# fallenshock/SinDDM

Hardware: AMD Instinct MI355X
Metric: diffusion steps/sec (finest scale) + imgs/sec full multi-scale sample, 1/2/4/8 GPU (higher is better)
Workload: dtype f32 (3x3 convs: binary16 hi/lo split products -- Winograd-domain GEMMs with all 4 MFMA terms, fp32 accumulate; fp32-equivalent, error vs float64 = the fp32 oracle's: tests/test_gpu_h2.py; everything else fp32); 1 GPU; C3: 6-scale pyramid, T=1000, finest scale 411x512, batch 64 per GPU, dim=160; batch_per_gpu=64, global_batch=64, scale=5, parallelism=independent chains over 1 GPU(s), one all-gather of the images

## Files before the change

include/sinddm_hip_debug.h:

```cpp
#ifndef SINDDM_HIP_DEBUG_H
#define SINDDM_HIP_DEBUG_H

#include <stddef.h>
#include <stdint.h>

#ifdef __cplusplus
extern "C" {
#endif

int sinddm_prof_begin(void);
int sinddm_prof_end(double* conv_ms_total, int64_t* conv_launches, double* conv_flops_total);
int sinddm_prof_end2(double* conv_ms_total, int64_t* conv_launches, double* conv_flops_total,
                     double* conv_exec_flops_total);
int sinddm_prof_end3(int kind, double* ms_total, int64_t* launches, double* flops_total,
                     double* exec_flops_total, int reset);

int sinddm_debug_routes(int dim_arg, int train, int B, int H, int W, int out[16]);

#define SINDDM_FWD_PLAN_BLOCK0 24
#define SINDDM_FWD_PLAN_BLOCK_INTS 14
#define SINDDM_FWD_PLAN_INTS (SINDDM_FWD_PLAN_BLOCK0 + 4 * SINDDM_FWD_PLAN_BLOCK_INTS)
#define SINDDM_FWD_PLAN_INTS_EXT (SINDDM_FWD_PLAN_INTS + 4)
int sinddm_debug_forward_plan(int dim_arg, int train, int B, int H, int W, int ncu, int64_t* out, int cap);

int sinddm_debug_first_conv(int variant, int ncu, int B, int H, int W, int Wt, int Cout, const float* in, const float* weights,
                            const float* bias, float* out, float* amax_out, void* stream);

int sinddm_debug_conv_path(int dim, int B, int H, int W);

int sinddm_debug_infer_path(int dim, int B, int H, int W);

int sinddm_debug_head_path(int dim, int B, int H, int W);
int sinddm_debug_head_offsets(int dim, int64_t out[3]);
int sinddm_debug_head(const float* packed, const float* g, const float* x_in, float* eps_out, int dim, int B, int H, int W,
                      int Wp, void* stream);

int sinddm_debug_train_path(int dim, int B, int H, int W);

int sinddm_debug_conv_wh(int variant, int ncu, int B, int H, int W, int Wt, int Cin, int Cout, int act, const float* in,
                         const float* weights, const float* bias, const float* resid, const float* aux, float* out,
                         float* out_pre, float* amax_out, void* scratch, size_t scratch_bytes, void* stream);
size_t sinddm_debug_conv_wh_scratch_bytes(int Cin, int Cout, int B);

int sinddm_debug_block_train(const float* params, const float* packed, const float* packed_bwd, int dim, int l,
                             const float* x, const float* cond_bias, const float* grad_y, float* y, float* grad_x,
                             float* grad_params, float* dcond, int B, int H, int W, void* ws, size_t ws_bytes,
                             void* stream);

int sinddm_debug_wgrad_map(int Cin, int Cout, int64_t ntiles, int ncu, uint32_t* wg_out, int wg_cap, int32_t* splits_out,
                           int splits_cap);

#define SINDDM_DWGRAD_TILES 6
#define SINDDM_DWGRAD_ROWS 7
int sinddm_debug_wgrad_plan(int taps, int Cin, int Cout, int B, int H, int W, int have_scr, int have_amax, int ncu, int out[4]);
int sinddm_debug_wgrad(int taps, int Cin, int Cout, int B, int H, int W, int ncu, int have_scr, int use_amax, const float* dout,
                       const float* in, float* gw, float* gb, void* scratch, size_t scratch_bytes, int plan_out[4], void* stream);
size_t sinddm_debug_wgrad_scratch_bytes(int taps, int Cin, int Cout, int B);
int sinddm_debug_wgrad_routes(int dim_arg, int B, int H, int W, int ncu, int* out, int cap);

// ... 5 lines not shown
```

sinddm_amd/_lib.py:

```python
from __future__ import annotations

import ctypes as C
import os
from typing import Optional

import torch

_HERE = os.path.dirname(os.path.abspath(__file__))
LIB_PATH = os.path.join(_HERE, "libsinddm_hip.so")

ABI_SYMBOLS = (
    "sinddm_abi_version", "sinddm_param_count", "sinddm_param_tensors", "sinddm_param_offset",
    "sinddm_packed_count", "sinddm_workspace_bytes", "sinddm_pack_weights", "sinddm_net_forward",
    "sinddm_q_sample", "sinddm_reverse_step", "sinddm_reverse_step_edit", "sinddm_upsample_bilinear", "sinddm_prof_begin", "sinddm_prof_end", "sinddm_prof_end2", "sinddm_prof_end3", "sinddm_debug_wgrad_map", "sinddm_debug_conv_path",
    "sinddm_debug_block_train", "sinddm_debug_infer_path", "sinddm_debug_train_path",
    "sinddm_train_workspace_bytes", "sinddm_packed_bwd_count", "sinddm_pack_weights_bwd",
    "sinddm_net_forward_train", "sinddm_net_backward", "sinddm_l1_loss_fwd_bwd", "sinddm_adam_ema_step",
    "sinddm_cond_embed", "sinddm_cond_stride", "sinddm_sample_chain", "sinddm_sample_chain2", "sinddm_sample_chain_ex",
    "sinddm_normal_fill", "sinddm_wrap_halo", "sinddm_upsample_bilinear_wrap", "sinddm_sample_chain_tile",
    "sinddm_sample_chain_keep", "sinddm_reverse_step_keep", "sinddm_normal_fill_samples", "sinddm_sample_chain_seeds",
    "sinddm_debug_head_path", "sinddm_debug_head_offsets", "sinddm_debug_head", "sinddm_debug_routes",
    "sinddm_debug_forward_plan",
    "sinddm_debug_wgrad_routes", "sinddm_debug_wgrad_plan", "sinddm_debug_wgrad", "sinddm_debug_wgrad_scratch_bytes",
    "sinddm_sample_chain_resample", "sinddm_reverse_step_jump",
    "sinddm_sample_chain_layout", "sinddm_layout_delta", "sinddm_reverse_step_layout",
    "sinddm_sample_chain_batch",
    "sinddm_sample_chain_solver", "sinddm_reverse_step_ms",
    "sinddm_q_sample_wrap", "sinddm_l1_loss_crop_fwd_bwd",
    "sinddm_sample_chain_mix", "sinddm_normal_fill_mix",
    "sinddm_l1_loss_weighted_fwd_bwd",
    "sinddm_debug_conv_wh", "sinddm_debug_conv_wh_scratch_bytes",
    "sinddm_debug_first_conv",
    "sinddm_patch_nnf_workspace_bytes", "sinddm_patch_nnf",
    "sinddm_q_sample_crop", "sinddm_l1_loss_rect_fwd_bwd",
    "sinddm_sample_chain_gate", "sinddm_reverse_step_keep_gate",
    "sinddm_patch_nnf_scaled_workspace_bytes", "sinddm_patch_nnf_scaled", "sinddm_patch_vote",
    "sinddm_score_workspace_bytes", "sinddm_score_chain",
    "sinddm_normal_fill_window",
)


ABI_VERSION = 3
DIM_FP32_CONVS = 0x10000
JUMP_STREAM = 1 << 31
MIX_MAX = 4
SCORE_MAX_EVALS = 1024
TILE_HALO = 16


class StepCoefs(C.Structure):
    _fields_ = [("mode", C.c_int), ("clip", C.c_int),
                ("sqrt_recip_ac_t", C.c_float), ("sqrt_recipm1_ac_t", C.c_float),
                ("coef1_t", C.c_float), ("coef2_t", C.c_float),
                ("gamma_t", C.c_float), ("gamma_tm1", C.c_float),
                ("sqrt_ac_tm1", C.c_float), ("sqrt_ac_t", C.c_float), ("sqrt_1m_ac_t", C.c_float),
                ("sqrt_1m_ac_tm1_mvar", C.c_float), ("sigma", C.c_float)]


class ChainOpts(C.Structure):
    _fields_ = [("edit_w", C.c_void_p), ("edit_c", C.c_void_p), ("noise", C.c_void_p)]


class KeepOpts(C.Structure):
    _fields_ = [("mask", C.c_void_p), ("x0", C.c_void_p), ("ab", C.POINTER(C.c_float))]

# ... 95 lines not shown
        "sinddm_normal_fill_window": (i, [p, i, p, i, i, i, p, i, i, p, p, i, p]),
        "sinddm_reverse_step_ms": (i, [p, p, p, p, p, C.POINTER(StepCoefs), f, p, p, p, p, p, f, f, i, i, i, p]),
        "sinddm_layout_delta": (i, [p, p, p, p, p, C.POINTER(StepCoefs), p, p, i, i, i, i, i, i, p]),
        "sinddm_reverse_step_layout": (i, [p, p, p, p, p, C.POINTER(StepCoefs), p, f, i, p, p, p, p, f, f, i, i, i, i, i, i, i,
                                           p]),
        "sinddm_reverse_step_jump": (i, [p, p, p, p, p, p, C.POINTER(StepCoefs), C.POINTER(JumpCoefs), p, p, p, p, f, f, i, i, i,
                                         p]),
        "sinddm_normal_fill_samples": (i, [p, i, i64, p, C.c_uint64, p]),
        "sinddm_reverse_step_keep": (i, [p, p, p, p, p, C.POINTER(StepCoefs), p, p, p, p, f, f, i, i, i, p]),
        "sinddm_reverse_step_keep_gate": (i, [p, p, p, p, p, C.POINTER(StepCoefs), p, p, p, p, f, f, i, i, i, p, f]),
        "sinddm_wrap_halo": (i, [p, p, i, i, i, i, i, p]),
        "sinddm_upsample_bilinear_wrap": (i, [p, p, i, i, i, i, i, i, i, p]),
        "sinddm_normal_fill": (i, [p, i64, C.c_uint64, C.c_uint64, p]),
        "sinddm_upsample_bilinear": (i, [p, p, i, i, i, i, i, p]),
        "sinddm_prof_begin": (i, []),
        "sinddm_prof_end": (i, [C.POINTER(C.c_double), C.POINTER(C.c_int64), C.POINTER(C.c_double)]),
        "sinddm_prof_end2": (i, [C.POINTER(C.c_double), C.POINTER(C.c_int64), C.POINTER(C.c_double),
                                 C.POINTER(C.c_double)]),
        "sinddm_prof_end3": (i, [i, C.POINTER(C.c_double), C.POINTER(C.c_int64), C.POINTER(C.c_double),
                                 C.POINTER(C.c_double), i]),
        "sinddm_debug_wgrad_map": (i, [i, i, i64, i, C.POINTER(C.c_uint32), i, C.POINTER(C.c_int32), i]),
        "sinddm_debug_conv_path": (i, [i, i, i, i]),
        "sinddm_debug_infer_path": (i, [i, i, i, i]),
        "sinddm_debug_train_path": (i, [i, i, i, i]),
        "sinddm_debug_head_path": (i, [i, i, i, i]),
        "sinddm_debug_routes": (i, [i, i, i, i, i, C.POINTER(C.c_int)]),
        "sinddm_debug_wgrad_routes": (i, [i, i, i, i, i, C.POINTER(C.c_int), i]),
        "sinddm_debug_wgrad_plan": (i, [i, i, i, i, i, i, i, i, i, C.POINTER(C.c_int)]),
        "sinddm_debug_wgrad": (i, [i, i, i, i, i, i, i, i, i, p, p, p, p, p, sz, C.POINTER(C.c_int), p]),
        "sinddm_debug_wgrad_scratch_bytes": (sz, [i, i, i, i]),
        "sinddm_debug_conv_wh": (i, [i, i, i, i, i, i, i, i, i, p, p, p, p, p, p, p, p, p, sz, p]),
        "sinddm_debug_conv_wh_scratch_bytes": (sz, [i, i, i]),
        "sinddm_debug_first_conv": (i, [i, i, i, i, i, i, i, p, p, p, p, p, p]),
        "sinddm_debug_head_offsets": (i, [i, C.POINTER(C.c_int64)]),
        "sinddm_debug_forward_plan": (i, [i, i, i, i, i, i, C.POINTER(C.c_int64), i]),
        "sinddm_debug_head": (i, [p, p, p, p, i, i, i, i, i, p]),
        "sinddm_debug_block_train": (i, [p, p, p, i, i, p, p, p, p, p, p, p, i, i, i, p, sz, p]),
        "sinddm_train_workspace_bytes": (sz, [i, i, i, i]),
        "sinddm_packed_bwd_count": (i64, [i]),
        "sinddm_pack_weights_bwd": (i, [p, p, i, p]),
        "sinddm_net_forward_train": (i, [p, p, p, p, i, f, p, i, i, i, i, p, sz, p]),
        "sinddm_net_backward": (i, [p, p, p, p, p, p, p, i, i, i, i, p, sz, p]),
        "sinddm_l1_loss_fwd_bwd": (i, [p, p, p, p, i64, f, p]),
        "sinddm_l1_loss_crop_fwd_bwd": (i, [p, p, p, p, i, i, i, i, i, f, p]),
        "sinddm_l1_loss_weighted_fwd_bwd": (i, [p, p, p, p, p, i, i, i, i, i, i, f, f, p]),
        "sinddm_q_sample_crop": (i, [p, p, p, p, p, p, p, p, i, p, i, i, i, i, i, i, p]),
        "sinddm_l1_loss_rect_fwd_bwd": (i, [p, p, p, p, p, p, p, i, i, i, i, i, i, f, f, p]),
        "sinddm_adam_ema_step": (i, [p, p, p, p, p, f, f, f, f, f, f, f, i, i64, p]),
        "sinddm_patch_nnf_workspace_bytes": (sz, [i, i, i, i, i, i, i, i]),
        "sinddm_patch_nnf": (i, [p, i, p, i, p, p, p, i, i, i, i, i, i, i, i, p, sz, p]),
        "sinddm_patch_nnf_scaled_workspace_bytes": (sz, [i, i, i, i, i, i, i, i]),
        "sinddm_patch_nnf_scaled": (i, [p, i, p, i, p, p, i, p, p, i, i, i, i, i, i, i, i, p, sz, p]),
        "sinddm_patch_vote": (i, [p, p, i, p, p, i, p, i, i, i, i, i, i, i, i, f, p]),
        "sinddm_score_workspace_bytes": (sz, [i, i, i, i, i]),
        "sinddm_score_chain": (i, [p, p, p, p, p, p, p, p, C.POINTER(C.c_int), i, f, C.c_uint64, C.c_uint64, p, p, i, i, i, i,
                                   p, sz, p, C.POINTER(ScoreOpts)]),
    }
    for name, (res, args) in sig.items():
        if not hasattr(lib, name):
            continue
        fn = getattr(lib, name)
        fn.restype = res
        fn.argtypes = args
    _lib = lib
    return lib

# ... 25 lines not shown
```

sinddm_amd/csrc/fwd_plan.h:

```cpp
#ifndef SINDDM_FWD_PLAN_H
#define SINDDM_FWD_PLAN_H
#include "common.h"

namespace sinddm {

enum ConvKernel { CONV_DIRECT = 0, CONV_C3 = 1, CONV_WINO2 = 2, CONV_WINO3 = 3, CONV_WINO4 = 4, CONV_WH = 8 };
ConvKernel conv3x3_route(const NetPlan& P, const Conv3x3Images& c, int B, int H, int W, bool have_amax, bool first_conv, int ncu);

enum FwdMode { FWD_INFER = 0, FWD_TRAIN = 1 };

enum ResidForm { RESID_NONE = 0, RESID_IDENTITY = 1, RESID_FUSED_DIRECT = 2, RESID_1X1_FRONT = 3 };
enum DwKernel { DW_TILES = 0, DW_ROWS = 1 };
#ifndef SINDDM_DW_ROWS
#define SINDDM_DW_ROWS 1
#endif
inline bool dw_rows_applies(int pi, int po) { return SINDDM_DW_ROWS && pi % 4 == 0 && po == pi && pi >= 192; }

enum LastLaunch {
    LAST_HEAD_STEP_PITCH = 0,
    LAST_HEAD_STEP = 1,
    LAST_HEAD_EPS = 2,
    LAST_FINAL_STEP_PITCH = 3,
    LAST_FINAL_PITCH = 4,
    LAST_FINAL_STEP = 5,
    LAST_FINAL = 6
};

struct FwdBlock {
    int wh_variant[2];
    int c3_variant;
    int amax_dw;
    int amax_in[2];
    int amax_out1;
    bool max_pass;
    ResidForm resid;
    bool bias_plain;
    DwKernel dw;
    int dw_pi, dw_po;
};

struct ForwardPlan {
    FwdMode mode;
    int B, H, W, ncu;
    int Wp, Wt, HW;
    bool padded;
    int route[8];
    bool any_wh;
    bool head;
    FwdBlock blk[4];
    LastLaunch last[2];
    unsigned last_gx[2];
    bool fuse_tail;
    bool rows_aligned;
    size_t off_cond, off_amax, off_buf[4], off_xpad, core_bytes;
    size_t cond_bytes() const { return off_buf[0]; }
    long long conv_items;
    int n_launches;
};

constexpr int CHAIN_COND_ROWS = 1024;

ForwardPlan forward_plan(const NetPlan& P, FwdMode mode, int B, int H, int W, int ncu);

// ... 32 lines not shown
    return first_conv && c.K == 3 && SINDDM_CONV_C3 ? CONV_C3 : CONV_DIRECT;
}

ForwardPlan forward_plan(const NetPlan& P, FwdMode mode, int B, int H, int W, int ncu) {
    const auto align256 = [](size_t v) { return (v + 255) / 256 * 256; };
    const bool train = mode == FWD_TRAIN;
    ForwardPlan F{};
    F.mode = mode; F.B = B; F.H = H; F.W = W; F.ncu = ncu;
    F.Wp = (!train && W % 4 != 0 && plan_pads_rows(P)) ? (W + 3) / 4 * 4 : W;
    F.padded = F.Wp != W;
    F.Wt = F.padded ? W : 0;
    F.HW = H * W;
    F.head = SINDDM_HEAD_COLLAPSE && !train && F.Wp % 4 == 0 && (long long)H * F.Wp < (1LL << 28);
    for (int l = 0; l < 4; ++l) {
        F.route[2 * l] = conv3x3_route(P, P.blk[l].c1, B, H, F.Wp, true, true, ncu);
        F.route[2 * l + 1] = F.head && l == 3 ? -1 : conv3x3_route(P, P.blk[l].c2, B, H, F.Wp, true, false, ncu);
        F.any_wh = F.any_wh || F.route[2 * l] == CONV_WH || F.route[2 * l + 1] == CONV_WH;
    }
    F.n_launches = (F.any_wh ? 1 : 0) + (F.padded ? 1 : 0) + 1;
    for (int l = 0; l < 4; ++l) {
        const BlockPlan& b = P.blk[l];
        FwdBlock& f = F.blk[l];
        const int r1 = F.route[2 * l], r2 = F.route[2 * l + 1];
        const bool wha = r1 == CONV_WH, whb = r2 == CONV_WH;
        const int variant = !train && conv_wr_pays(B, H, F.Wp, b.cout, ncu) ? 2 : 1;
        f.wh_variant[0] = wha ? variant : 0;
        f.wh_variant[1] = whb ? variant : 0;
        f.c3_variant = r1 != CONV_C3 ? 0 : !train && c3m_pays(B, H, F.Wp, b.cout, ncu) ? 2 : 1;
        f.amax_dw = f.amax_in[0] = wha ? 2 * l : -1;
        f.amax_in[1] = whb ? 2 * l + 1 : -1;
        f.amax_out1 = whb && (wha || r1 == CONV_C3) ? 2 * l + 1 : -1;
        f.max_pass = whb && f.amax_out1 < 0;
        f.resid = r2 < 0 ? RESID_NONE : b.nchr == 0 ? RESID_IDENTITY : r2 == CONV_DIRECT ? RESID_FUSED_DIRECT : RESID_1X1_FRONT;
        f.bias_plain = wha;
        f.dw_pi = f.dw_po = F.Wp;
        f.dw = dw_rows_applies(f.dw_pi, f.dw_po) ? DW_ROWS : DW_TILES;
        F.n_launches += 2 + (f.max_pass ? 1 : 0) + (r2 >= 0 ? 1 : 0) + (f.resid == RESID_1X1_FRONT ? 1 : 0);
    }
    const unsigned row_quads = (unsigned)((H * (F.Wp / 4) + 255) / 256);
    F.fuse_tail = F.HW % 4 == 0 || F.padded;
    F.rows_aligned = F.HW % 4 == 0 && !F.padded;
    if (F.head || F.padded) {
        F.last[1] = F.head ? (F.padded ? LAST_HEAD_STEP_PITCH : LAST_HEAD_STEP) : LAST_FINAL_STEP_PITCH;
        F.last[0] = F.head ? LAST_HEAD_EPS : LAST_FINAL_PITCH;
        F.last_gx[0] = F.last_gx[1] = row_quads;
    } else {
        F.last[0] = LAST_FINAL;
        F.last_gx[0] = (unsigned)(((F.HW + 3) / 4 + 255) / 256);
        F.last[1] = F.fuse_tail ? LAST_FINAL_STEP : LAST_FINAL;
        F.last_gx[1] = F.fuse_tail ? (unsigned)((F.HW / 4 + 255) / 256) : F.last_gx[0];
    }
    F.conv_items = (long long)B * ((F.Wp + 31) / 32) * ((H + 7) / 8) * 2;
    if (!train) {
        const size_t amax = align256((size_t)B * AMAX_STRIDE * sizeof(float));
        const size_t rows = B > CHAIN_COND_ROWS ? B : CHAIN_COND_ROWS;
        const size_t act = align256((size_t)B * P.dim * H * F.Wp * sizeof(float));
        F.off_cond = 0;
        F.off_amax = align256(rows * P.cond_stride * sizeof(float));
        for (int i = 0; i < 4; ++i) F.off_buf[i] = F.off_amax + amax + i * act;
        F.off_xpad = F.off_buf[3] + act;
        F.core_bytes = F.off_xpad + (F.padded ? align256((size_t)B * CHANNELS * H * F.Wp * sizeof(float)) : 0);
    }
    return F;
}

}
// ... 2 lines not shown
```

sinddm_amd/csrc/sinddm_fwd.hip:

```cpp
#include "conv_mfma.h"
#include "conv_wino4.h"
#include "conv_wh.h"
#include "conv_c3m.h"
#include "internal.h"
#include "step_tail.h"
#include "chain_run.h"
#include <type_traits>
namespace sinddm {

ConvProfiler& conv_profiler() {
    static ConvProfiler p;
    return p;
}

__global__ void pack_kernel(const float* __restrict__ params, float* __restrict__ packed, PackArgs a) {
    long long i = (long long)blockIdx.x * blockDim.x + threadIdx.x;
    if (i >= a.total) return;
    int s = 0;
    long long base = 0;
    while (s < a.nseg - 1 && i >= base + a.seg[s].count) { base += a.seg[s].count; ++s; }
    const PackSeg& g = a.seg[s];
    const long long j = i - base;
    float v = 0.0f;
    if (g.kind == 0) {
// ... 773 lines not shown
                           io.x_tilde, io.out, t, extra..., span, io.chw, io.hw);
    });
    return hipGetLastError() != hipSuccess ? SINDDM_E_BADARG : 0;
}
#define TAIL_KERNEL(name) \
    [](auto E, auto N, auto K) { return &name<decltype(E)::value, decltype(N)::value, decltype(K)::value>; }

static HeadEps head_eps(const NetPlan& P, const float* packed, const float* g, const float* xin, int H, int Wp) {
    return HeadEps{g, xin, packed + P.pk_hc, packed + P.pk_hr, packed + P.pk_hb, P.half, P.dim, H, Wp};
}

int conv3x3_launch(ConvKernel k, const Conv3x3Images& c, const float* packed, ConvArgs a, hipStream_t st, int wh_variant) {
    a.coblks = c.coblks;
    switch (k) {
        case CONV_WH:
            a.w3 = packed + c.wh; a.wsinv = packed + c.wh_sinv;
            if (wh_variant != 1 && wh_variant != 2) return SINDDM_E_BADARG;
            return conv_wh_launch(a, st, wh_variant);
        case CONV_WINO4:
        case CONV_WINO3:
            a.w3 = packed + c.wino24; a.nch3 = conv3x3_nchw(c);
            return k == CONV_WINO4 ? conv_wino4_launch(a, st) : conv_wino3_launch(a, st);
        case CONV_WINO2:
            if (a.Cin % 4 != 0) return SINDDM_E_BADSHAPE;
            a.w3 = packed + c.wino2; a.nch3 = conv3x3_nchw(c);
            return conv_wino2_launch(a, c.mt, st);
        case CONV_DIRECT:
            a.w3 = packed + c.direct; a.nch3 = conv3x3_nch(c);
            return conv_launch(a, c.mt, st);
        default: return SINDDM_E_BADARG;
    }
}

int block_forward(const NetPlan& P, const ForwardPlan& F, int l, const float* params, const float* packed, const float* cur,
                  const float* cond, int cond_stride, float* hbuf, float* gbuf, float* obuf, float* upre, hipStream_t st,
                  float* amax) {
    const BlockPlan& b = P.blk[l];
    const FwdBlock& f = F.blk[l];
    const int B = F.B, H = F.H, W = F.Wp, Wt = F.Wt;
    const ConvKernel k1 = (ConvKernel)F.route[2 * l], k2 = (ConvKernel)F.route[2 * l + 1];
    if ((f.amax_dw >= 0 || f.amax_in[1] >= 0) && !amax) return SINDDM_E_BADARG;
    auto slot = [&](int i) { return i >= 0 ? amax + i : nullptr; };
    int rc = dwconv_launch(cur, params + b.dw_w, params + b.dw_b, cond, cond_stride, nullptr, 0, hbuf, B, b.cin, H,
                           Wt > 0 ? Wt : W, st, f.dw_pi, f.dw_po, slot(f.amax_dw));
    if (rc) return rc;
    if (k1 == CONV_C3 && f.c3_variant == 2) {
        if (upre) return SINDDM_E_BADARG;
        rc = conv_c3m_launch(hbuf, params + b.c1_w, params + b.c1_b, gbuf, B, H, W, b.cout, Wt, slot(f.amax_out1), st);
    } else if (k1 == CONV_C3) {
        rc = conv_c3_valu_launch(hbuf, params + b.c1_w, params + b.c1_b, gbuf, upre, B, H, W, b.cout, Wt, slot(f.amax_out1), st);
    } else {
        ConvArgs c1{};
        c1.in = hbuf; c1.out = gbuf; c1.out_pre = upre;
        c1.B = B; c1.H = H; c1.W = W; c1.Cin = b.cin; c1.Cout = b.cout;
        c1.act = 1; c1.zero = packed + P.pk_zero; c1.Wt = Wt;
        c1.bias = f.bias_plain ? params + b.c1_b : packed + b.pk_b1;
        c1.amax_in = slot(f.amax_in[0]); c1.amax_out = slot(f.amax_out1);
        rc = conv3x3_launch(k1, b.c1, packed, c1, st, f.wh_variant[0]);
    }
    if (rc || f.resid == RESID_NONE) return rc;
    if (f.max_pass) {
        rc = amax_tensor_launch(gbuf, slot(f.amax_in[1]), B, (long long)b.cout * H * W, st);
        if (rc) return rc;
    }
    ConvArgs c2{};
    c2.in = gbuf; c2.out = obuf;
    c2.B = B; c2.H = H; c2.W = W; c2.Cin = b.cout; c2.Cout = b.cout;
    c2.act = 0; c2.zero = packed + P.pk_zero; c2.Wt = Wt;
    c2.bias = packed + b.pk_b2;
    c2.amax_in = slot(f.amax_in[1]);
    if (f.resid == RESID_IDENTITY) c2.resid = cur;
    else if (f.resid == RESID_FUSED_DIRECT) {
        c2.in2 = cur; c2.Cin2 = b.cin; c2.w1 = packed + b.pk_res; c2.nch1 = b.nchr;
    } else {
        ConvArgs r1{};
        r1.in2 = cur; r1.Cin2 = b.cin; r1.w1 = packed + b.pk_res; r1.nch1 = b.nchr; r1.nch3 = 0;
        r1.bias = packed + b.pk_b2; r1.out = obuf; r1.Cout = b.cout; r1.coblks = b.coblks;
        r1.B = B; r1.H = H; r1.W = W; r1.zero = packed + P.pk_zero;
        rc = conv1x1_launch(r1, b.mt, st);
        if (rc) return rc;
        c2.resid = obuf; c2.bias = nullptr;
    }
    return conv3x3_launch(k2, b.c2, packed, c2, st, f.wh_variant[1]);
}

bool wh_enabled() { return SINDDM_CONV_WH != 0; }
int wh_pack(const Conv3x3Images& c, const float* w, float* packed, int transpose, hipStream_t st) {
    if (c.wh < 0) return 0;
    return wh_pack_launch(w, packed + c.wh_sinv, packed + c.wh, transpose ? c.M : c.K, transpose ? c.K : c.M, transpose, st);
}

__global__ __launch_bounds__(256) void amax_tensor_kernel(const float* __restrict__ x, float* __restrict__ amax, long long n4) {
    const int b = blockIdx.y;
    const f32x4* p = reinterpret_cast<const f32x4*>(x) + (size_t)b * n4;
    float m = 0.f;
    for (long long i = (long long)blockIdx.x * 256 + threadIdx.x; i < n4; i += (long long)gridDim.x * 256) {
        const f32x4 v = p[i];
        m = fmaxf(m, fmaxf(fmaxf(fabsf(v.x), fabsf(v.y)), fmaxf(fabsf(v.z), fabsf(v.w))));
    }
    amax_publish(m, amax + (size_t)b * AMAX_STRIDE);
}
int amax_tensor_launch(const float* x, float* amax, int B, long long per_sample, hipStream_t st) {
    if (per_sample % 4 != 0) return SINDDM_E_BADSHAPE;
    const long long n4 = per_sample / 4;
    long long bx = (n4 + 2047) / 2048;
    const long long cap = (8LL * cu_count() + B - 1) / B;
    if (bx > cap) bx = cap;
    if (bx < 1) bx = 1;
    hipLaunchKernelGGL(amax_tensor_kernel, dim3((unsigned)bx, B), dim3(256), 0, st, x, amax, n4);
    SINDDM_LAUNCH_CHECK();
    return 0;
}
// ... 373 lines not shown
    const float* cond_row;
    float* cur;
    float* nxt;
    TailArgs t;
    bool jump, pull, ms;
    JumpArgs jp;
    float g;
    float q;
};

static int chain_split(ChainCtx& k) {
    const ChainRun& r = k.r;
    const NetPlan& p = k.p;
    const int B = r.B, H = k.c.H, W = k.c.W;
    ChainSplit& s = k.sp;
    const ForwardPlan& whole = k.fp;
    const long long items = whole.conv_items, ncu = whole.ncu;
    const long long rounds = (items + ncu - 1) / ncu;
    bool split = k.sx != nullptr && k.sx != k.st && B >= 2 && whole.fuse_tail && r.n_steps > 0 && items < SINDDM_SPLIT_ITEMS_HI * ncu &&
                 items >= SINDDM_SPLIT_ITEMS_LO * ncu && (rounds * ncu - items) * 25 >= rounds * ncu;
    if (split && whole.route[5] == CONV_WH) split = false;
    s = ChainSplit{};
    s.Bh[0] = B;
    s.fp[0] = whole;
    s.wsh[0] = static_cast<char*>(r.ws); s.wsz[0] = r.ws_bytes;
    if (split) {
        const ForwardPlan h0 = forward_plan(p, FWD_INFER, (B + 1) / 2, H, W, whole.ncu), h1 = forward_plan(p, FWD_INFER, B - (B + 1) / 2, H, W, whole.ncu);
        split = whole.cond_bytes() + h0.core_bytes + h1.core_bytes <= r.ws_bytes;
        if (split) {
            s.on = true;
            s.Bh[0] = h0.B; s.Bh[1] = h1.B;
            s.fp[0] = h0; s.fp[1] = h1;
            for (int l = 0; l < 4; ++l) s.fp[0].blk[l].c3_variant = s.fp[1].blk[l].c3_variant = whole.blk[l].c3_variant;
            s.wsh[0] = static_cast<char*>(r.ws) + whole.cond_bytes(); s.wsz[0] = h0.core_bytes;
            s.wsh[1] = s.wsh[0] + s.wsz[0]; s.wsz[1] = h1.core_bytes;
            if (hipEventCreateWithFlags(&s.ev_go, hipEventDisableTiming) != hipSuccess) return SINDDM_E_BADARG;
            if (hipEventCreateWithFlags(&s.ev_done, hipEventDisableTiming) != hipSuccess) {
                (void)hipEventDestroy(s.ev_go);
                return SINDDM_E_BADARG;
            }
        }
    }
    s.hoff = (size_t)s.Bh[0] * CHANNELS * H * W;
    return 0;
}

static int chain_half_step(const ChainCtx& k, const ChainStepPlan& s, int h) {
    const ChainRun& r = k.r;
    const int H = k.c.H, W = k.c.W, Bn = k.sp.Bh[h];
    const size_t o = h ? k.sp.hoff : 0;
    hipStream_t st = h ? k.sx : k.st;
    ChainStep cs{};
    cs.plan = &k.sp.fp[h];
    cs.cond_row = s.cond_row;
    cs.x_tilde = r.x_tilde ? r.x_tilde + o : nullptr; cs.x_next = k.fp.fuse_tail && !s.jump && !s.pull && !s.ms ? s.nxt + o : nullptr;
    cs.tail = s.t;
    const int b0 = cs.tail.b0 = h ? k.sp.Bh[0] : 0;
    if (k.c.sseeds) cs.tail.sseeds = k.c.sseeds + b0;
    if (k.c.mkeys) {
        cs.tail.mkeys = k.c.mkeys + (size_t)b0 * k.c.mK;
        cs.tail.mw = k.c.mw + (size_t)b0 * k.c.mK;
    }
    cs.tail.ew = batch_slice(s.t.ew, b0, s.t.sew); cs.tail.ec = batch_slice(s.t.ec, b0, s.t.sec);
    cs.tail.km = batch_slice(s.t.km, b0, s.t.skm); cs.tail.kx = batch_slice(s.t.kx, b0, s.t.skx);
    int rc = net_forward_impl(k.p, r.params, r.packed, s.cur + o, nullptr, r.t_list[s.i], r.scale, r.eps + o, Bn, H, W, k.sp.wsh[h],
                              k.sp.wsz[h], st, nullptr, &cs);
// ... 442 lines not shown
    return sinddm_prof_end3(0, conv_ms_total, conv_launches, conv_flops_total, conv_exec_flops_total, 1);
}

int sinddm_debug_infer_path(int dim, int B, int H, int W) {
    int r[16];
    const int rc = sinddm_debug_routes(dim, 0, B, H, W, r);
    return rc ? rc : r[5];
}

int sinddm_debug_head_path(int dim, int B, int H, int W) {
    NetPlan p = make_plan(dim);
    if (!p.ok || B <= 0 || H <= 0 || W <= 0) return SINDDM_E_BADARG;
    return forward_plan(p, FWD_INFER, B, H, W, cu_count()).head ? 1 : 0;
}

int sinddm_debug_forward_plan(int dim_arg, int train, int B, int H, int W, int ncu, int64_t* out, int cap) {
    NetPlan p = make_plan(dim_arg);
    if (!p.ok || !out || cap < SINDDM_FWD_PLAN_INTS || B <= 0 || H <= 0 || W <= 0) return SINDDM_E_BADARG;
    if (ncu <= 0) ncu = cu_count();
    const ForwardPlan F = forward_plan(p, train ? FWD_TRAIN : FWD_INFER, B, H, W, ncu);
    const int64_t head[SINDDM_FWD_PLAN_BLOCK0] = {
        F.Wp, F.padded, F.Wt, F.HW, F.head, F.any_wh, F.fuse_tail, F.rows_aligned, F.last[0], F.last_gx[0], F.last[1], F.last_gx[1],
        F.n_launches, F.conv_items, (int64_t)F.off_cond, (int64_t)F.off_amax, (int64_t)F.off_buf[0], (int64_t)F.off_buf[1],
        (int64_t)F.off_buf[2], (int64_t)F.off_buf[3], (int64_t)F.off_xpad, (int64_t)F.core_bytes,
        train ? 0 : (int64_t)chain_workspace_bytes(F, forward_plan(p, FWD_INFER, (B + 1) / 2, H, W, ncu)), F.ncu};
    for (int i = 0; i < SINDDM_FWD_PLAN_BLOCK0; ++i) out[i] = head[i];
    for (int l = 0; l < 4; ++l) {
        const FwdBlock& f = F.blk[l];
        const int64_t blk[SINDDM_FWD_PLAN_BLOCK_INTS] = {F.route[2 * l], F.route[2 * l + 1], f.wh_variant[0], f.wh_variant[1], f.amax_dw,
                                                         f.amax_in[0], f.amax_out1, f.max_pass, f.amax_in[1], f.resid, f.bias_plain,
                                                         f.dw, f.dw_pi, f.dw_po};
        for (int i = 0; i < SINDDM_FWD_PLAN_BLOCK_INTS; ++i) out[SINDDM_FWD_PLAN_BLOCK0 + l * SINDDM_FWD_PLAN_BLOCK_INTS + i] = blk[i];
        if (cap >= SINDDM_FWD_PLAN_INTS_EXT) out[SINDDM_FWD_PLAN_INTS + l] = f.c3_variant;
    }
    return 0;
}

int sinddm_debug_first_conv(int variant, int ncu, int B, int H, int W, int Wt, int Cout, const float* in, const float* weights,
                            const float* bias, float* out, float* amax_out, void* stream) {
    if (!in || !weights || !bias || !out || variant < 0 || variant > 2 || B <= 0 || H <= 0 || W <= 0 || Cout <= 0)
        return SINDDM_E_BADARG;
    if (B > 65535 || (long long)H * W >= (1LL << 28) || (long long)Cout * H * W >= (1LL << 31)) return SINDDM_E_BADSHAPE;
    if (Wt != 0 && (Wt > W || Wt <= W - 4)) return SINDDM_E_BADSHAPE;
    if (variant == 2 && !c3m_applies(B, H, W, Cout)) return SINDDM_E_BADSHAPE;
    if (ncu <= 0) ncu = cu_count();
    if (variant == 0) variant = c3m_pays(B, H, W, Cout, ncu) ? 2 : 1;
    hipStream_t st = static_cast<hipStream_t>(stream);
    if (variant == 2) {
        if ((uintptr_t)out % 16 != 0) return SINDDM_E_BADARG;
        return conv_c3m_launch(in, weights, bias, out, B, H, W, Cout, Wt, amax_out, st, ncu);
    }
    return conv_c3_valu_launch(in, weights, bias, out, nullptr, B, H, W, Cout, Wt, amax_out, st);
}

int sinddm_debug_head_offsets(int dim, int64_t out[3]) {
    NetPlan p = make_plan(dim);
    if (!p.ok || !out) return SINDDM_E_BADARG;
    out[0] = p.pk_hc; out[1] = p.pk_hr; out[2] = p.pk_hb;
    return 0;
}

int sinddm_debug_head(const float* packed, const float* g, const float* x_in, float* eps_out, int dim, int B, int H, int W,
                      int Wp, void* stream) {
    if (!packed || !g || !x_in || !eps_out || B <= 0 || H <= 0 || W <= 0) return SINDDM_E_BADARG;
    NetPlan p = make_plan(dim);
    if (!p.ok) return SINDDM_E_BADSHAPE;
    if (Wp % 4 != 0 || W > Wp || W <= Wp - 4 || (long long)H * Wp >= (1LL << 28) || B > 65535) return SINDDM_E_BADSHAPE;
    hipLaunchKernelGGL(head_eps_kernel, dim3((unsigned)((H * (Wp / 4) + 255) / 256), B), dim3(256), 0,
                       static_cast<hipStream_t>(stream), head_eps(p, packed, g, x_in, H, Wp), eps_out, W);
    SINDDM_LAUNCH_CHECK();
    return 0;
}

static size_t wh_debug_round(size_t v) { return (v + 255) / 256 * 256; }
static bool wh_debug_shape_ok(int Cin, int Cout, int B) { return B >= 1 && B <= 65535 && wh_plan_ok(Cin, Cout) && Cout >= 80; }

size_t sinddm_debug_conv_wh_scratch_bytes(int Cin, int Cout, int B) {
    if (!wh_debug_shape_ok(Cin, Cout, B)) return 0;
    return wh_debug_round((size_t)wh_image_halfs(Cin, Cout) * 2) + wh_debug_round((size_t)Cout * sizeof(float)) +
           wh_debug_round((size_t)B * AMAX_STRIDE * sizeof(float));
}

int sinddm_debug_conv_wh(int variant, int ncu, int B, int H, int W, int Wt, int Cin, int Cout, int act, const float* in,
                         const float* weights, const float* bias, const float* resid, const float* aux, float* out,
                         float* out_pre, float* amax_out, void* scratch, size_t scratch_bytes, void* stream) {
// ... 51 lines not shown

int sinddm_upsample_bilinear(const float* in, float* out, int BC, int h, int w, int H, int W, void* stream) {
    if (!in || !out || BC <= 0 || h <= 0 || w <= 0 || H <= 0 || W <= 0) return SINDDM_E_BADARG;
    const float sy = (float)h / (float)H, sx = (float)w / (float)W;
    hipLaunchKernelGGL((upsample_bilinear_kernel<false, false>), dim3((H * W + 255) / 256, BC), dim3(256), 0,
                       static_cast<hipStream_t>(stream), in, out, h, w, H, W, sy, sx);
    SINDDM_LAUNCH_CHECK();
    return 0;
}

int sinddm_upsample_bilinear_wrap(const float* in, float* out, int BC, int h, int w, int H, int W, int wrap_y, int wrap_x,
                                  void* stream) {
    if (!in || !out || BC <= 0 || h <= 0 || w <= 0 || H <= 0 || W <= 0) return SINDDM_E_BADARG;
    const float sy = (float)h / (float)H, sx = (float)w / (float)W;
    const dim3 grid((H * W + 255) / 256, BC);
    hipStream_t st = static_cast<hipStream_t>(stream);
    if (wrap_y && wrap_x) hipLaunchKernelGGL((upsample_bilinear_kernel<true, true>), grid, dim3(256), 0, st, in, out, h, w, H, W, sy, sx);
    else if (wrap_y) hipLaunchKernelGGL((upsample_bilinear_kernel<true, false>), grid, dim3(256), 0, st, in, out, h, w, H, W, sy, sx);
    else if (wrap_x) hipLaunchKernelGGL((upsample_bilinear_kernel<false, true>), grid, dim3(256), 0, st, in, out, h, w, H, W, sy, sx);
    else hipLaunchKernelGGL((upsample_bilinear_kernel<false, false>), grid, dim3(256), 0, st, in, out, h, w, H, W, sy, sx);
    SINDDM_LAUNCH_CHECK();
    return 0;
}

int sinddm_wrap_halo(float* ext, const float* src, int BC, int H, int W, int halo_y, int halo_x, void* stream) {
    if (!ext || BC <= 0 || H <= 0 || W <= 0 || halo_y < 0 || halo_x < 0 || halo_y > (1 << 20) || halo_x > (1 << 20))
        return SINDDM_E_BADARG;
    return wrap_halo_launch(ext, src, BC, H, W, halo_y, halo_x, static_cast<hipStream_t>(stream));
}

}

#include "window_fill.h"
```

Measured before the change: 804.5 sample-steps/s (finest scale, batch x steps/s, all GPUs).

## Add bf16 triple-split MFMA kernel for residual 1x1 projection convs

```diff
diff --git a/include/sinddm_hip_debug.h b/include/sinddm_hip_debug.h
--- a/include/sinddm_hip_debug.h
+++ b/include/sinddm_hip_debug.h
@@ -21,10 +21,14 @@
 #define SINDDM_FWD_PLAN_BLOCK_INTS 14
 #define SINDDM_FWD_PLAN_INTS (SINDDM_FWD_PLAN_BLOCK0 + 4 * SINDDM_FWD_PLAN_BLOCK_INTS)
 #define SINDDM_FWD_PLAN_INTS_EXT (SINDDM_FWD_PLAN_INTS + 4)
+#define SINDDM_FWD_PLAN_INTS_EXT2 (SINDDM_FWD_PLAN_INTS_EXT + 4)
 int sinddm_debug_forward_plan(int dim_arg, int train, int B, int H, int W, int ncu, int64_t* out, int cap);
 
 int sinddm_debug_first_conv(int variant, int ncu, int B, int H, int W, int Wt, int Cout, const float* in, const float* weights,
                             const float* bias, float* out, float* amax_out, void* stream);
+
+int sinddm_debug_conv1x1(int variant, int ncu, int B, int H, int W, int Cin, int Cout, const float* in, const float* weights,
+                         const float* bias, float* out, void* stream);
 
 int sinddm_debug_conv_path(int dim, int B, int H, int W);
 
diff --git a/sinddm_amd/_lib.py b/sinddm_amd/_lib.py
--- a/sinddm_amd/_lib.py
+++ b/sinddm_amd/_lib.py
@@ -30,7 +30,7 @@
     "sinddm_sample_chain_mix", "sinddm_normal_fill_mix",
     "sinddm_l1_loss_weighted_fwd_bwd",
     "sinddm_debug_conv_wh", "sinddm_debug_conv_wh_scratch_bytes",
-    "sinddm_debug_first_conv",
+    "sinddm_debug_first_conv", "sinddm_debug_conv1x1",
     "sinddm_patch_nnf_workspace_bytes", "sinddm_patch_nnf",
     "sinddm_q_sample_crop", "sinddm_l1_loss_rect_fwd_bwd",
     "sinddm_sample_chain_gate", "sinddm_reverse_step_keep_gate",
@@ -192,6 +192,7 @@
         "sinddm_debug_conv_wh": (i, [i, i, i, i, i, i, i, i, i, p, p, p, p, p, p, p, p, p, sz, p]),
         "sinddm_debug_conv_wh_scratch_bytes": (sz, [i, i, i]),
         "sinddm_debug_first_conv": (i, [i, i, i, i, i, i, i, p, p, p, p, p, p]),
+        "sinddm_debug_conv1x1": (i, [i, i, i, i, i, i, i, p, p, p, p, p]),
         "sinddm_debug_head_offsets": (i, [i, C.POINTER(C.c_int64)]),
         "sinddm_debug_forward_plan": (i, [i, i, i, i, i, i, C.POINTER(C.c_int64), i]),
         "sinddm_debug_head": (i, [p, p, p, p, i, i, i, i, i, p]),
diff --git a/sinddm_amd/csrc/conv1x1_b3.h b/sinddm_amd/csrc/conv1x1_b3.h
--- /dev/null
+++ b/sinddm_amd/csrc/conv1x1_b3.h
@@ -0,0 +1,216 @@
+#pragma once
+#include "conv_args.h"
+#include "fwd_plan.h"
+
+namespace sinddm {
+
+constexpr int B3_THREADS = 512;
+constexpr int B3_PIX = 256;
+constexpr int B3_MTW = 5;
+constexpr int B3_MTT = 10;
+
+using bf16x8 = __attribute__((ext_vector_type(8))) __bf16;
+using u32x4 = __attribute__((ext_vector_type(4))) unsigned;
+
+inline size_t proj_b3_lds_bytes(int cin) { return (size_t)((cin + 31) / 32) * B3_MTT * 3 * 64 * 16 + B3_MTT * 16 * sizeof(float); }
+
+__device__ __forceinline__ unsigned b3_cvt_pk(float lo, float hi) {
+    unsigned r;
+    asm("v_cvt_pk_bf16_f32 %0, %1, %2" : "=v"(r) : "v"(lo), "v"(hi));
+    return r;
+}
+__device__ __forceinline__ void b3_split2(float x0, float x1, unsigned& p1, unsigned& p2, unsigned& p3) {
+    p1 = b3_cvt_pk(x0, x1);
+    float r0 = x0 - __builtin_bit_cast(float, p1 << 16), r1 = x1 - __builtin_bit_cast(float, p1 & 0xffff0000u);
+    p2 = b3_cvt_pk(r0, r1);
+    r0 -= __builtin_bit_cast(float, p2 << 16);
+    r1 -= __builtin_bit_cast(float, p2 & 0xffff0000u);
+    p3 = b3_cvt_pk(r0, r1);
+}
+
+template <int NKS>
+__global__ __launch_bounds__(B3_THREADS) void conv1x1_b3_kernel(ConvArgs p, int tiles_per_img, int ntiles) {
+    extern __shared__ __attribute__((aligned(16))) float smem[];
+    bf16x8* const sw = reinterpret_cast<bf16x8*>(smem);
+    float* const sbias = smem + NKS * B3_MTT * 3 * 64 * 4;
+    const int tid = threadIdx.x, lane = tid & 63;
+    const int wave = __builtin_amdgcn_readfirstlane(tid >> 6);
+    const int seg = wave & 3, mhalf = wave >> 2;
+    const int l16 = lane & 15, kq = lane >> 4;
+    const int HW = p.H * p.W;
+    const int Cin = p.Cin2;
+    constexpr int CO_LDS = ConvCfg<5, 4>::CO_LDS;
+    constexpr unsigned OOB = 0x40000000u;
+
+    for (int e = tid; e < NKS * B3_MTT * 64; e += B3_THREADS) {
+        const int l = e & 63, q = e >> 6;
+        const int ks = q / B3_MTT, mt = q - ks * B3_MTT;
+        const int co = mt * 16 + (l & 15), cb = co / 80, col = co - cb * 80;
+        const int ci0 = 32 * ks + 8 * (l >> 4);
+        float w[8];
+#pragma unroll
+        for (int j = 0; j < 8; ++j)
+            w[j] = ci0 + j < Cin ? p.w1[((size_t)cb * p.nch1 * KC + ci0 + j) * CO_LDS + col] : 0.f;
+        u32x4 w1, w2, w3;
+#pragma unroll
+        for (int j = 0; j < 4; ++j) {
+            unsigned q1, q2, q3;
+            b3_split2(w[2 * j], w[2 * j + 1], q1, q2, q3);
+            w1[j] = q1; w2[j] = q2; w3[j] = q3;
+        }
+        sw[(q * 3 + 0) * 64 + l] = __builtin_bit_cast(bf16x8, w1);
+        sw[(q * 3 + 1) * 64 + l] = __builtin_bit_cast(bf16x8, w2);
+        sw[(q * 3 + 2) * 64 + l] = __builtin_bit_cast(bf16x8, w3);
+    }
+    for (int e = tid; e < B3_MTT * 16; e += B3_THREADS) sbias[e] = p.bias ? p.bias[e] : 0.f;
+    __syncthreads();
+
+    struct TileCtx {
+        __amdgpu_buffer_rsrc_t rs;
+        unsigned pxo;
+    };
+    auto make_ctx = [&](int tile) {
+        TileCtx c;
+        const bool live = tile < ntiles;
+        const int b = live ? tile / tiles_per_img : 0;
+        const int p0 = (tile - b * tiles_per_img) * B3_PIX;
+        const int px = p0 + seg * 64 + l16 * 4;
+        c.rs = __builtin_amdgcn_make_buffer_rsrc(const_cast<float*>(p.in2 + (size_t)b * Cin * HW), 0, live ? Cin * HW * 4 : 0,
+                                                 0x00020000);
+        c.pxo = px < HW ? (unsigned)px * 4u : OOB;
+        return c;
+    };
+    const unsigned kqo = (unsigned)(8 * kq * HW) * 4u;
+    auto load_b = [&](const TileCtx& c, int ks, f32x4 (&v)[8]) {
+        unsigned base = 32 * ks + 8 * kq < Cin ? c.pxo + kqo : OOB;
+        asm volatile("" : "+v"(base));
+#pragma unroll
+        for (int j = 0; j < 8; ++j) {
+            const unsigned o = base + (unsigned)((32 * ks + j) * HW) * 4u;
+            v[j] = __builtin_bit_cast(f32x4, __builtin_amdgcn_raw_buffer_load_b128(c.rs, (int)o, 0, 0));
+        }
+    };
+
+    bf16x8 x1[4], x2[4], x3[4];
+    auto split_b = [&](const f32x4 (&v)[8]) {
+#pragma unroll
+        for (int nt = 0; nt < 4; ++nt) {
+            u32x4 a, b2, c;
+#pragma unroll
+            for (int j = 0; j < 4; ++j) {
+                unsigned q1, q2, q3;
+                b3_split2(v[2 * j][nt], v[2 * j + 1][nt], q1, q2, q3);
+                a[j] = q1; b2[j] = q2; c[j] = q3;
+            }
+            x1[nt] = __builtin_bit_cast(bf16x8, a);
+            x2[nt] = __builtin_bit_cast(bf16x8, b2);
+            x3[nt] = __builtin_bit_cast(bf16x8, c);
+        }
+    };
+    TileCtx ctx = make_ctx(blockIdx.x);
+    {
+        f32x4 first[8];
+        load_b(ctx, 0, first);
+        split_b(first);
+    }
+
+    for (int tile = blockIdx.x; tile < ntiles; tile += gridDim.x) {
+        const int b = tile / tiles_per_img;
+        const int p0 = (tile - b * tiles_per_img) * B3_PIX;
+        const int px0 = p0 + seg * 64 + l16 * 4;
+        const TileCtx nctx = make_ctx(tile + gridDim.x);
+        f32x4 acc[B3_MTW][4];
+#pragma unroll
+        for (int mt = 0; mt < B3_MTW; ++mt)
+#pragma unroll
+            for (int nt = 0; nt < 4; ++nt) acc[mt][nt] = f32x4{0.f, 0.f, 0.f, 0.f};
+
+#pragma unroll
+        for (int ks = 0; ks < NKS; ++ks) {
+            f32x4 nxt[8];
+            if (ks + 1 < NKS) load_b(ctx, ks + 1, nxt);
+            else load_b(nctx, 0, nxt);
+            const bf16x8* wk = sw + ((ks * B3_MTT + mhalf * B3_MTW) * 3) * 64 + lane;
+            bf16x8 wa[2][3];
+#pragma unroll
+            for (int i = 0; i < 3; ++i) wa[0][i] = wk[i * 64];
+            __builtin_amdgcn_sched_barrier(0);
+#pragma unroll
+            for (int mt = 0; mt < B3_MTW; ++mt) {
+                if (mt + 1 < B3_MTW) {
+#pragma unroll
+                    for (int i = 0; i < 3; ++i) wa[(mt + 1) & 1][i] = wk[((mt + 1) * 3 + i) * 64];
+                }
+                __builtin_amdgcn_sched_barrier(0);
+                const bf16x8 w1 = wa[mt & 1][0], w2 = wa[mt & 1][1], w3 = wa[mt & 1][2];
+#pragma unroll
+                for (int nt = 0; nt < 4; ++nt) acc[mt][nt] = __builtin_amdgcn_mfma_f32_16x16x32_bf16(w1, x3[nt], acc[mt][nt], 0, 0, 0);
+#pragma unroll
+                for (int nt = 0; nt < 4; ++nt) acc[mt][nt] = __builtin_amdgcn_mfma_f32_16x16x32_bf16(w3, x1[nt], acc[mt][nt], 0, 0, 0);
+#pragma unroll
+                for (int nt = 0; nt < 4; ++nt) acc[mt][nt] = __builtin_amdgcn_mfma_f32_16x16x32_bf16(w2, x2[nt], acc[mt][nt], 0, 0, 0);
+#pragma unroll
+                for (int nt = 0; nt < 4; ++nt) acc[mt][nt] = __builtin_amdgcn_mfma_f32_16x16x32_bf16(w1, x2[nt], acc[mt][nt], 0, 0, 0);
+#pragma unroll
+                for (int nt = 0; nt < 4; ++nt) acc[mt][nt] = __builtin_amdgcn_mfma_f32_16x16x32_bf16(w2, x1[nt], acc[mt][nt], 0, 0, 0);
+#pragma unroll
+                for (int nt = 0; nt < 4; ++nt) acc[mt][nt] = __builtin_amdgcn_mfma_f32_16x16x32_bf16(w1, x1[nt], acc[mt][nt], 0, 0, 0);
+                __builtin_amdgcn_sched_barrier(0);
+            }
+            split_b(nxt);
+            __builtin_amdgcn_sched_barrier(0);
+        }
+
+        const __amdgpu_buffer_rsrc_t rs_out = __builtin_amdgcn_make_buffer_rsrc(p.out + (size_t)b * p.Cout * HW, 0,
+                                                                                (unsigned)(p.Cout * HW) * 4u, 0x00020000);
+#pragma unroll
+        for (int mt = 0; mt < B3_MTW; ++mt) {
+            const int c0 = (mhalf * B3_MTW + mt) * 16 + kq * 4;
+            const f32x4 bias4 = *reinterpret_cast<const f32x4*>(sbias + c0);
+#pragma unroll
+            for (int r = 0; r < 4; ++r) {
+                f32x4 v{acc[mt][0][r], acc[mt][1][r], acc[mt][2][r], acc[mt][3][r]};
+                v += bias4[r];
+                unsigned o = px0 < HW ? (unsigned)((c0 + r) * HW + px0) * 4u : OOB;
+                asm volatile("" : "+v"(o));
+                __builtin_amdgcn_raw_buffer_store_b128(__builtin_bit_cast(u32x4, v), rs_out, (int)o, 0, 0);
+            }
+        }
+        ctx = nctx;
+    }
+}
+
+int conv1x1_b3_launch(const ConvArgs& a, int ncu, hipStream_t st) {
+    if (!proj_b3_applies(a.B, a.H, a.W, a.Cin2, a.Cout) || a.resid || a.act != 0) return SINDDM_E_BADSHAPE;
+    if ((uintptr_t)a.in2 % 16 != 0 || (uintptr_t)a.out % 16 != 0) return SINDDM_E_BADARG;
+    ConvProfiler& prof = conv_profiler();
+    const bool rec = prof.begin(st);
+    const int HW = a.H * a.W;
+    const int tpi = (HW + B3_PIX - 1) / B3_PIX;
+    const int ntiles = a.B * tpi;
+    if (ncu <= 0) ncu = cu_count();
+    const unsigned grid = (unsigned)(ntiles < ncu ? ntiles : ncu);
+    const size_t lds = proj_b3_lds_bytes(a.Cin2);
+#define B3_GO(NKS)                                                                                                        \
+    do {                                                                                                                  \
+        static const hipError_t attr_rc = hipFuncSetAttribute(reinterpret_cast<const void*>(&conv1x1_b3_kernel<NKS>),     \
+                                                              hipFuncAttributeMaxDynamicSharedMemorySize,                 \
+                                                              (int)proj_b3_lds_bytes(32 * NKS));                          \
+        if (attr_rc != hipSuccess) return (int)attr_rc;                                                                   \
+        hipLaunchKernelGGL((conv1x1_b3_kernel<NKS>), dim3(grid), dim3(B3_THREADS), lds, st, a, tpi, ntiles);              \
+    } while (0)
+    switch ((a.Cin2 + 31) / 32) {
+        case 1: B3_GO(1); break;
+        case 2: B3_GO(2); break;
+        default: B3_GO(3);
+    }
+#undef B3_GO
+    if (rec) {
+        const double fl = 2.0 * a.B * a.H * a.W * (double)a.Cout * (double)a.Cin2;
+        prof.end(st, 2, fl, 6.0 * fl * (double)((a.Cin2 + 31) / 32 * 32) / (double)a.Cin2);
+    }
+    SINDDM_LAUNCH_CHECK();
+    return 0;
+}
+
+}
diff --git a/sinddm_amd/csrc/fwd_plan.h b/sinddm_amd/csrc/fwd_plan.h
--- a/sinddm_amd/csrc/fwd_plan.h
+++ b/sinddm_amd/csrc/fwd_plan.h
@@ -16,6 +16,22 @@
 #endif
 inline bool dw_rows_applies(int pi, int po) { return SINDDM_DW_ROWS && pi % 4 == 0 && po == pi && pi >= 192; }
 
+#ifndef SINDDM_PROJ_B3
+#define SINDDM_PROJ_B3 1
+#endif
+inline bool proj_b3_applies(int B, int H, int W, int cin, int cout) {
+    const long long hw = (long long)H * W;
+    return SINDDM_PROJ_B3 && B > 0 && cout == 160 && cin >= 8 && cin % 8 == 0 && cin <= 96 && hw % 4 == 0 &&
+           cout * hw * 4 < 0x40000000LL && (long long)B * ((hw + 255) / 256 + 1) * 256 < 0x40000000LL;
+}
+constexpr int SINDDM_PROJ_B3_MIN_PIXELS = 3072;
+constexpr int SINDDM_PROJ_B3_MAX_PIXELS = 12032;
+inline bool proj_b3_pays(int B, int H, int W, int cin, int cout, int ncu) {
+    (void)ncu;
+    const long long hw = (long long)H * W;
+    return proj_b3_applies(B, H, W, cin, cout) && hw >= SINDDM_PROJ_B3_MIN_PIXELS && hw <= SINDDM_PROJ_B3_MAX_PIXELS;
+}
+
 enum LastLaunch {
     LAST_HEAD_STEP_PITCH = 0,
     LAST_HEAD_STEP = 1,
@@ -29,6 +45,7 @@
 struct FwdBlock {
     int wh_variant[2];
     int c3_variant;
+    int proj_variant;
     int amax_dw;
     int amax_in[2];
     int amax_out1;
@@ -127,6 +144,7 @@
         f.amax_out1 = whb && (wha || r1 == CONV_C3) ? 2 * l + 1 : -1;
         f.max_pass = whb && f.amax_out1 < 0;
         f.resid = r2 < 0 ? RESID_NONE : b.nchr == 0 ? RESID_IDENTITY : r2 == CONV_DIRECT ? RESID_FUSED_DIRECT : RESID_1X1_FRONT;
+        f.proj_variant = f.resid != RESID_1X1_FRONT ? 0 : !train && !P.fp32_convs && proj_b3_pays(B, H, F.Wp, b.cin, b.cout, ncu) ? 2 : 1;
         f.bias_plain = wha;
         f.dw_pi = f.dw_po = F.Wp;
         f.dw = dw_rows_applies(f.dw_pi, f.dw_po) ? DW_ROWS : DW_TILES;
diff --git a/sinddm_amd/csrc/sinddm_fwd.hip b/sinddm_amd/csrc/sinddm_fwd.hip
--- a/sinddm_amd/csrc/sinddm_fwd.hip
+++ b/sinddm_amd/csrc/sinddm_fwd.hip
@@ -829,6 +829,7 @@
     }
 }
 
+int conv1x1_b3_launch(const ConvArgs& a, int ncu, hipStream_t st);
 int block_forward(const NetPlan& P, const ForwardPlan& F, int l, const float* params, const float* packed, const float* cur,
                   const float* cond, int cond_stride, float* hbuf, float* gbuf, float* obuf, float* upre, hipStream_t st,
                   float* amax) {
@@ -874,7 +875,8 @@
         r1.in2 = cur; r1.Cin2 = b.cin; r1.w1 = packed + b.pk_res; r1.nch1 = b.nchr; r1.nch3 = 0;
         r1.bias = packed + b.pk_b2; r1.out = obuf; r1.Cout = b.cout; r1.coblks = b.coblks;
         r1.B = B; r1.H = H; r1.W = W; r1.zero = packed + P.pk_zero;
-        rc = conv1x1_launch(r1, b.mt, st);
+        if (f.proj_variant != 1 && f.proj_variant != 2) return SINDDM_E_BADARG;
+        rc = f.proj_variant == 2 ? conv1x1_b3_launch(r1, F.ncu, st) : conv1x1_launch(r1, b.mt, st);
         if (rc) return rc;
         c2.resid = obuf; c2.bias = nullptr;
     }
@@ -1314,6 +1316,7 @@
             s.Bh[0] = h0.B; s.Bh[1] = h1.B;
             s.fp[0] = h0; s.fp[1] = h1;
             for (int l = 0; l < 4; ++l) s.fp[0].blk[l].c3_variant = s.fp[1].blk[l].c3_variant = whole.blk[l].c3_variant;
+            for (int l = 0; l < 4; ++l) s.fp[0].blk[l].proj_variant = s.fp[1].blk[l].proj_variant = whole.blk[l].proj_variant;
             s.wsh[0] = static_cast<char*>(r.ws) + whole.cond_bytes(); s.wsz[0] = h0.core_bytes;
             s.wsh[1] = s.wsh[0] + s.wsz[0]; s.wsz[1] = h1.core_bytes;
             if (hipEventCreateWithFlags(&s.ev_go, hipEventDisableTiming) != hipSuccess) return SINDDM_E_BADARG;
@@ -1822,6 +1825,7 @@
                                                          f.dw, f.dw_pi, f.dw_po};
         for (int i = 0; i < SINDDM_FWD_PLAN_BLOCK_INTS; ++i) out[SINDDM_FWD_PLAN_BLOCK0 + l * SINDDM_FWD_PLAN_BLOCK_INTS + i] = blk[i];
         if (cap >= SINDDM_FWD_PLAN_INTS_EXT) out[SINDDM_FWD_PLAN_INTS + l] = f.c3_variant;
+        if (cap >= SINDDM_FWD_PLAN_INTS_EXT2) out[SINDDM_FWD_PLAN_INTS_EXT + l] = f.proj_variant;
     }
     return 0;
 }
@@ -1841,6 +1845,42 @@
         return conv_c3m_launch(in, weights, bias, out, B, H, W, Cout, Wt, amax_out, st, ncu);
     }
     return conv_c3_valu_launch(in, weights, bias, out, nullptr, B, H, W, Cout, Wt, amax_out, st);
+}
+
+int sinddm_debug_conv1x1(int variant, int ncu, int B, int H, int W, int Cin, int Cout, const float* in, const float* weights,
+                         const float* bias, float* out, void* stream) {
+    if (!in || !weights || !bias || !out || variant < 0 || variant > 2 || B <= 0 || H <= 0 || W <= 0 || Cin <= 0 || Cout <= 0)
+        return SINDDM_E_BADARG;
+    if (B > 65535 || Cout % 80 != 0 || Cout > 160 || Cin > 160 || (long long)Cin * H * W * 4 >= 0x40000000LL ||
+        (long long)Cout * H * W * 4 >= 0x40000000LL || (long long)B * ((H * W + 255) / 256 + 1) * 256 >= 0x40000000LL)
+        return SINDDM_E_BADSHAPE;
+    if (variant == 2 && !proj_b3_applies(B, H, W, Cin, Cout)) return SINDDM_E_BADSHAPE;
+    if ((uintptr_t)in % 16 != 0 || (uintptr_t)out % 16 != 0) return SINDDM_E_BADARG;
+    if (ncu <= 0) ncu = cu_count();
+    if (variant == 0) variant = proj_b3_pays(B, H, W, Cin, Cout, ncu) ? 2 : 1;
+    hipStream_t st = static_cast<hipStream_t>(stream);
+    const int mt = 5, coblks = Cout / 80;
+    PackArgs a{};
+    pack_add_direct(a, 0, 0, Cin, Cout, 1, mt, coblks, 0);
+    const long long zero = a.total;
+    PackSeg z{};
+    z.kind = 2; z.dst = zero; z.count = 64;
+    a.seg[a.nseg++] = z;
+    a.total += z.count;
+    float* img = nullptr;
+    hipError_t e = hipMalloc(reinterpret_cast<void**>(&img), (size_t)a.total * sizeof(float));
+    if (e != hipSuccess) return (int)e;
+    int rc = pack_launch(weights, img, a, st);
+    if (!rc) {
+        ConvArgs r1{};
+        r1.in2 = in; r1.Cin2 = Cin; r1.w1 = img; r1.nch1 = (Cin + KC - 1) / KC; r1.nch3 = 0;
+        r1.bias = bias; r1.out = out; r1.Cout = Cout; r1.coblks = coblks;
+        r1.B = B; r1.H = H; r1.W = W; r1.zero = img + zero;
+        rc = variant == 2 ? conv1x1_b3_launch(r1, ncu, st) : conv1x1_launch(r1, mt, st);
+    }
+    e = hipStreamSynchronize(st);
+    (void)hipFree(img);
+    return rc ? rc : (int)e;
 }
 
 int sinddm_debug_head_offsets(int dim, int64_t out[3]) {
@@ -1958,3 +1998,4 @@
 }
 
 #include "window_fill.h"
+#include "conv1x1_b3.h"
```

Result: no change. 800.3 sample-steps/s (finest scale, batch x steps/s, all GPUs) (-0.5%).
